# AIM-Harvard/pyradiomics

Measured on NVIDIA H100. Metric: voxels/s full-texture voxel-based, higher is better.
Workload: dtype f64

## Files before the change

### pyradiomics_b200/csrc/glcm_fast.cuh

```cuda
#pragma once
#include "vox_features.cuh"
#include "straightline.inc"
#ifndef __CUDACC__
#include <algorithm>
using std::max;
using std::min;
#endif

#ifdef __CUDA_ARCH__
#define RB_CTZ(x) (__ffs((int)(x)) - 1)
#define RB_POPC(x) __popc((unsigned)(x))
#else
#define RB_CTZ(x) __builtin_ctz((unsigned)(x))
#define RB_POPC(x) __builtin_popcount((unsigned)(x))
#endif

#if (defined(__CUDA_ARCH__) || defined(RB_EMULATE_BLOCK)) && defined(RB_GLCM_BLOCK_SYNC)
#define RB_ANGLE_SYNC() __syncthreads()
#else
#define RB_ANGLE_SYNC() ((void)0)
#endif

namespace rb {

constexpr int GF_NA = 13;
constexpr int GF_LOGT = 40;
constexpr int GF_KT = 256;
constexpr int GF_DENSE_MAX_CLS = 10;

struct GlcmFastTables {
  uint8_t orig[GF_NA];
  uint8_t np[GF_NA];
  uint8_t pA[GF_NA][18], pB[GF_NA][18];
  double log2t[GF_LOGT];
  double idm[GF_KT], idmn[GF_KT], id[GF_KT], idn[GF_KT], inv[GF_KT];
  double lz0[19];
  double rsq[GF_LOGT];
};

static const double kLanczosStart0[19] = {0.47733602246716966, 0.56675833970975287, 1.047365457332734, 0.92625467075097456, 0.641109550601909, 0.58281392786638453, 0.84830875358718982, 0.43673418560371335, 0.9227560440146213, 1.1918028652699371, 0.49824571462957101, 1.1988811518333182, 0.91723745310037241, 0.34589793559411208, 0.69183966616781278, 1.1364799193275177, 0.9474534998820221, 0.57647286407011211, 0.9839281633300665};

inline void glcm_fast_build_tables(GlcmFastTables& T, int Ng) {
  int ang[13][3], k = 0;
  for (int z = 1; z >= -1; z--) for (int y = 1; y >= -1; y--) for (int x = 1; x >= -1; x--) {
    if (k < 13) { ang[k][0] = z; ang[k][1] = y; ang[k][2] = x; k++; }
  }
  int slot = 0;
  for (int want = 1; want <= 3; want++)
    for (int a = 0; a < 13; a++) {
      int nm = (ang[a][0] != 0) + (ang[a][1] != 0) + (ang[a][2] != 0);
      if (nm != want) continue;
      T.orig[slot] = (uint8_t)a;
      int n = 0;
      for (int z = 0; z < 3; z++) for (int y = 0; y < 3; y++) for (int x = 0; x < 3; x++) {
        int z2 = z + ang[a][0], y2 = y + ang[a][1], x2 = x + ang[a][2];
        if (z2 < 0 || z2 > 2 || y2 < 0 || y2 > 2 || x2 < 0 || x2 > 2) continue;
        T.pA[slot][n] = (uint8_t)(z * 9 + y * 3 + x);
        T.pB[slot][n] = (uint8_t)(z2 * 9 + y2 * 3 + x2);
        n++;
      }
      T.np[slot] = (uint8_t)n;
      for (int t = n; t < 18; t++) { T.pA[slot][t] = 0; T.pB[slot][t] = 0; }
      slot++;
    }
  for (int i = 0; i < 19; i++) T.lz0[i] = kLanczosStart0[i];
  T.log2t[0] = 0; T.rsq[0] = 0;
  for (int c = 1; c < GF_LOGT; c++) { T.log2t[c] = log2((double)c); T.rsq[c] = 1.0 / sqrt((double)c); }
  for (int d = 0; d < GF_KT; d++) {
    double kk = d;
    T.idm[d] = 1.0 / (1.0 + kk * kk);
    T.idmn[d] = 1.0 / (1.0 + kk * kk / ((double)Ng * Ng));
    T.id[d] = 1.0 / (1.0 + kk);
    T.idn[d] = 1.0 / (1.0 + kk / (double)Ng);
    T.inv[d] = d ? 1.0 / (kk * kk) : 0.0;
  }
}

struct GlcmSolveTables {
  uint8_t np[GF_NA];
  uint8_t pA[GF_NA][18], pB[GF_NA][18];
  double lz0[19];
  double rsq[GF_LOGT];
  double rinv[GF_LOGT];
  uint32_t lo_mask[GF_NA];
  uint8_t dshift[GF_NA];
};
RB_HD void glcm_solve_tables_from(const GlcmFastTables& T, GlcmSolveTables& S) {
  for (int a = 0; a < GF_NA; a++) {
    S.np[a] = T.np[a];
    for (int t = 0; t < 18; t++) { S.pA[a][t] = T.pA[a][t]; S.pB[a][t] = T.pB[a][t]; }
    uint32_t lo = 0;
    for (int t = 0; t < T.np[a]; t++) lo |= 1u << (T.pA[a][t] < T.pB[a][t] ? T.pA[a][t] : T.pB[a][t]);
    S.lo_mask[a] = lo;
    S.dshift[a] = (uint8_t)(T.pA[a][0] < T.pB[a][0] ? T.pB[a][0] - T.pA[a][0] : T.pA[a][0] - T.pB[a][0]);
  }
  for (int i = 0; i < 19; i++) S.lz0[i] = T.lz0[i];
  for (int i = 0; i < GF_LOGT; i++) { S.rsq[i] = T.rsq[i]; S.rinv[i] = i ? 1.0 / (double)i : 0.0; }
}

#ifdef __CUDA_ARCH__
#define RB_VCMPEQ4_LSB(a, b) (__vcmpeq4((a), (b)) & 0x01010101u)
#else
static inline uint32_t rb_vcmpeq4_lsb(uint32_t a, uint32_t b) {
  const uint32_t x = a ^ b;
  const uint32_t t = ((x & 0x7F7F7F7Fu) + 0x7F7F7F7Fu) | x | 0x7F7F7F7Fu;
  return (~t) >> 7;
}
#define RB_VCMPEQ4_LSB(a, b) rb_vcmpeq4_lsb((a), (b))
#endif

RB_HD void glcm_pack_window(const uint8_t* w, int ws, uint32_t* W7) {
#pragma unroll
  for (int k = 0; k < 7; k++) {
    uint32_t v = 0;
#pragma unroll
    for (int b = 0; b < 4; b++) if (4 * k + b < 27) v |= (uint32_t)w[(4 * k + b) * ws] << (8 * b);
    W7[k] = v;
  }
}
RB_HD uint32_t glcm_eq_positions(const uint32_t* W7, uint32_t lev) {
  const uint32_t rep = lev * 0x01010101u;
  uint32_t m = 0;
#pragma unroll
  for (int k = 0; k < 7; k++) m |= ((RB_VCMPEQ4_LSB(W7[k], rep) * 0x01020408u) >> 24) << (4 * k);
  return m & 0x7FFFFFFu;
}

template <int N>
RB_HD double tridiag_bisect_static(const double* d, const double* e, double lo, double hi, int k) {
  for (int it = 0; it < 36; it++) {
    const double xm = 0.5 * (lo + hi);
    double pm2 = 1.0, pm1 = d[0] - xm;
    int cnt = pm1 <= 0;
#pragma unroll
    for (int i = 1; i < N; i++) {
      const double e2 = e[i] * e[i];
      if (e2 == 0) { pm2 = 1.0; pm1 = d[i] - xm; cnt += pm1 <= 0; continue; }
      const double p = (d[i] - xm) * pm1 - e2 * pm2;
      const bool neg_prev = pm1 < 0 || (pm1 == 0 && pm2 > 0);
      const bool neg_cur = p < 0 || (p == 0 && !neg_prev);
      cnt += neg_cur != neg_prev;
      pm2 = pm1; pm1 = p;
    }
    if (cnt > k) hi = xm; else lo = xm;
  }
  return 0.5 * (lo + hi);
}
template <int N, bool SYNC>
RB_HD void tridiag_extreme_pair_static(const double* d, const double* e, double* hi_out, double* lo_out, bool live) {
  double lo = d[0], hi = d[0];
#pragma unroll
  for (int i = 0; i < N; i++) {
    const double r = (i > 0 ? fabs(e[i]) : 0.0) + (i + 1 < N ? fabs(e[i + 1]) : 0.0);
    lo = fmin(lo, d[i] - r); hi = fmax(hi, d[i] + r);
  }
  double x[2] = {hi + 1e-9, lo - 1e-9};
  bool done[2] = {!live, !live};
  for (int it = 0; it < 24; it++) {
    const bool pending = !(done[0] && done[1]);
#if defined(__CUDA_ARCH__) || defined(RB_EMULATE_BLOCK)
    if (SYNC) { if (!__syncthreads_or(pending)) break; } else
#endif
    if (!pending) break;
#pragma unroll
    for (int c = 0; c < 2; c++) {
      double p0 = 1.0, p1 = d[0] - x[c], q0 = 0.0, q1 = -1.0, r0 = 0.0, r1 = 0.0;
#pragma unroll
      for (int i = 1; i < N; i++) {
        const double a = d[i] - x[c], b = e[i] * e[i];
        const double p2 = a * p1 - b * p0;
        const double q2 = a * q1 - p1 - b * q0;
        const double r2 = a * r1 - 2.0 * q1 - b * r0;
        p0 = p1; p1 = p2; q0 = q1; q1 = q2; r0 = r1; r1 = r2;
      }
      if (done[c]) continue;
      if (p1 == 0) { done[c] = true; continue; }
      const double G = q1 / p1, H = G * G - r1 / p1;
      const double disc = (double)(N - 1) * ((double)N * H - G * G);
      const double sq = sqrt(disc > 0 ? disc : 0.0);
      const double den = fabs(G + sq) > fabs(G - sq) ? G + sq : G - sq;
      if (den == 0 || den != den) continue;
      const double step = (double)N / den;
      x[c] -= step;
      if (fabs(step) < 1e-10) done[c] = true;
    }
  }
  *hi_out = done[0] ? x[0] : tridiag_bisect_static<N>(d, e, lo - 1e-9, hi + 1e-9, N - 1);
  *lo_out = done[1] ? x[1] : tridiag_bisect_static<N>(d, e, lo - 1e-9, hi + 1e-9, 0);
  if (!live) { *hi_out = 0; *lo_out = 0; }
}

#if defined(__CUDA_ARCH__) || defined(RB_EMULATE_BLOCK)
#define RB_SOLVE_SYNC() do { if (SYNC) __syncthreads(); } while (0)
#else
#define RB_SOLVE_SYNC() do { } while (0)
#endif
template <int N, bool SYNC = false, class TT>
RB_HD double glcm_small_solve(const uint8_t* w, int ws, const uint32_t* W7, const TT& T, int s, bool* ok, bool live = true) {
  RB_SOLVE_SYNC();
  const int dsh = T.dshift[s];
  const uint32_t NZ = ~glcm_eq_positions(W7, 0u) & 0x7FFFFFFu;
  const uint32_t VL = NZ & (NZ >> dsh) & T.lo_mask[s];
  uint32_t U = VL | (VL << dsh);
  uint32_t El[N], Eh[N];
  int R[N];
#pragma unroll
  for (int i = 0; i < N; i++) {
    uint32_t E = 0;
    if (U) { E = glcm_eq_positions(W7, w[RB_CTZ(U) * ws]); U &= ~E; }
    El[i] = E & VL;
    Eh[i] = (E >> dsh) & VL;
    R[i] = RB_POPC(El[i]) + RB_POPC(Eh[i]);
  }
  *ok = U == 0;
  if (!SYNC && U) return 0.0;
  if (U) live = false;
  RB_SOLVE_SYNC();
  const double invS = 1.0 / (2.0 * RB_POPC(VL));
  double v1[N], rs[N];
#pragma unroll
  for (int i = 0; i < N; i++) { rs[i] = T.rsq[R[i]]; v1[i] = sqrt(R[i] * invS); }
  double a[N][N];
#pragma unroll
  for (int i = 0; i < N; i++)
#pragma unroll
    for (int j = 0; j <= i; j++) {
      const int c = (i == j) ? 2 * RB_POPC(El[i] & Eh[i]) : RB_POPC(El[i] & Eh[j]) + RB_POPC(El[j] & Eh[i]);
      a[i][j] = c * rs[i] * rs[j] - v1[i] * v1[j];
    }
  double d[N], e[N];
  e[0] = 0;
#pragma unroll
  for (int k = 0; k + 2 < N; k++) {
    RB_SOLVE_SYNC();
    double sigma = 0;
#pragma unroll
    for (int i = k + 2; i < N; i++) sigma += a[i][k] * a[i][k];
    const double x0 = a[k + 1][k];
    d[k] = a[k][k];
    if (sigma < 1e-30) { e[k + 1] = x0; continue; }
    const double nrm = sqrt(x0 * x0 + sigma);
    const double alpha = x0 > 0 ? -nrm : nrm;
    double v[N], pv[N];
    v[k + 1] = x0 - alpha;
#pragma unroll
    for (int i = k + 2; i < N; i++) v[i] = a[i][k];
    const double beta = -1.0 / (alpha * v[k + 1]);
    double K = 0;
#pragma unroll
    for (int i = k + 1; i < N; i++) {
      double acc = 0;
#pragma unroll
      for (int j = k + 1; j < N; j++) acc += (j <= i ? a[i][j] : a[j][i]) * v[j];
      pv[i] = beta * acc;
      K += v[i] * pv[i];
    }
    K *= 0.5 * beta;
#pragma unroll
    for (int i = k + 1; i < N; i++) pv[i] -= K * v[i];
#pragma unroll
    for (int i = k + 1; i < N; i++)
#pragma unroll
      for (int j = k + 1; j <= i; j++) a[i][j] -= v[i] * pv[j] + pv[i] * v[j];
    e[k + 1] = alpha;
  }
  d[N - 2] = a[N - 2][N - 2]; e[N - 1] = a[N - 1][N - 2]; d[N - 1] = a[N - 1][N - 1];
  double hi, lo;
  RB_SOLVE_SYNC();
  tridiag_extreme_pair_static<N, SYNC>(d, e, &hi, &lo, live);
  return fmax(fabs(hi), fabs(lo));
}

}
#include "glcm_lanczos.cuh"
namespace rb {

template <class TT>
RB_HD double glcm_lanczos_solve(const uint8_t* w, int ws, const TT& T, int s, int cls, double* sm, int st) {
  if (s > 2) return 1.0;
  int n = 0;
  double r;
  if (cls <= 12) r = glcm_lanczos_task<14>(w, ws, T, s, sm, st, &n);
  else if (cls <= 14) r = glcm_lanczos_task<16>(w, ws, T, s, sm, st, &n);
  else { r = glcm_lanczos_task<18>(w, ws, T, s, sm, st, &n); if (n == 19) r = 1.0; }
  return r;
}

template <class TT>
RB_HD double glcm_fast_solve(const uint8_t* w, int ws, const TT& T, int s, int cls) {
  if (cls <= GF_DENSE_MAX_CLS) {
    uint32_t W7[7];
    glcm_pack_window(w, ws, W7);
    bool ok = false;
    double r;
    if (cls <= 2) r = glcm_small_solve<4>(w, ws, W7, T, s, &ok);
    else if (cls <= 4) r = glcm_small_solve<6>(w, ws, W7, T, s, &ok);
    else if (cls <= 6) r = glcm_small_solve<8>(w, ws, W7, T, s, &ok);
    else if (cls <= 8) r = glcm_small_solve<10>(w, ws, W7, T, s, &ok);
    else r = glcm_small_solve<12>(w, ws, W7, T, s, &ok);
    return ok ? r : NAN;
  }
  double sm[LZ_NARR * 18];
  return glcm_lanczos_solve(w, ws, T, s, cls, sm, 1);
}

constexpr int GF_NCLS = 16, GF_CLS_BITS = 4;
RB_HD int glcm_task_class(int n) { return n <= 2 ? 0 : n >= 17 ? 15 : n - 2; }

struct GlcmAcc {
  double sum[GLCM_NF];
  int n_ok, n_imc2;
  uint32_t tasks;
  unsigned long long tcls;
  bool ja_nan;
};

#ifdef __CUDA_ARCH__
#define RB_VMINU2(a, b) __vminu2((a), (b))
#define RB_VMAXU2(a, b) __vmaxu2((a), (b))
#else
static inline uint32_t rb_vminu2(uint32_t a, uint32_t b) {
  return min(a >> 16, b >> 16) << 16 | min(a & 0xFFFFu, b & 0xFFFFu);
}
static inline uint32_t rb_vmaxu2(uint32_t a, uint32_t b) {
  return max(a >> 16, b >> 16) << 16 | max(a & 0xFFFFu, b & 0xFFFFu);
}
#define RB_VMINU2(a, b) rb_vminu2((a), (b))
#define RB_VMAXU2(a, b) rb_vmaxu2((a), (b))
#endif

template <int NP, bool FULL>
RB_HD void glcm_fast_angle(const uint8_t* w, int ws, const uint32_t* eq, int es,
                           const GlcmFastTables& T, int s, const VoxParams& P, GlcmAcc& acc) {
  const uint8_t* pA = T.pA[s];
  const uint8_t* pB = T.pB[s];
  const int dsh = (int)pB[0] - (int)pA[0];
  uint32_t key[NP];
  uint32_t valid = 0, EA = 0, EB = 0;
  int n = 0, Ssum = 0, Sab = 0, Sq = 0, Skd = 0;
  bool selfpair = false;
#pragma unroll
  for (int t = 0; t < NP; t++) {
    const int a = w[pA[t] * ws], b = w[pB[t] * ws];
    const bool ok = FULL || (a != 0 && b != 0);
    const int kd = a > b ? a - b : b - a, ks = a + b;
    key[t] = ok ? (uint32_t)(ks << 16 | kd) : 0xFFFFFFFFu;
    if (ok) {
      valid |= 1u << t; EA |= 1u << pA[t]; EB |= 1u << pB[t];
      n++; Ssum += ks; Sab += a * b; Sq += a * a + b * b; Skd += kd;
      selfpair |= kd == 0;
    }
  }
  const int orig = T.orig[s];
  if (!FULL && n == 0) {
    if (P.alive[orig >> 5] >> (orig & 31) & 1u) acc.ja_nan = true;
    return;
  }
  double rl = 0, lgE = 0;
  int E2 = 0, cmax = 0;
  uint32_t reps = 0, all = 0, comp = 0;
  uint32_t em[NP];
#pragma unroll
  for (int t = 0; t < NP; t++) {
    em[t] = 0;
    if (valid >> t & 1u) {
      const uint32_t ea = eq[pA[t] * es], eb = eq[pB[t] * es];
      rl += T.log2t[RB_POPC(ea & EA) + RB_POPC(ea & EB)] + T.log2t[RB_POPC(eb & EA) + RB_POPC(eb & EB)];
      reps |= (ea & (0u - ea)) | (eb & (0u - eb));
      em[t] = ea | eb;
      all |= em[t];
      if (!comp) comp = em[t];
      const int c = RB_POPC(((ea & (eb >> dsh)) | (eb & (ea >> dsh))) & EA);
      const int cc = ea == eb ? 2 * c : c;
      lgE += T.log2t[cc];
      E2 += 2 * cc;
      cmax = cc > cmax ? cc : cmax;
    }
  }
  const int nlev = RB_POPC(reps);
  double mcc;
  if (P.n_roi_levels < 2) mcc = 1.0;
  else if (nlev < 2) mcc = 0.0;
  else {
    for (int sweep = 0; sweep < NP; sweep++) {
      const uint32_t before = comp;
#pragma unroll
      for (int t = 0; t < NP; t++) if (em[t] & comp) comp |= em[t];
      if (comp == before) break;
    }
    bool bipartite = false;
    if (comp == all && !selfpair) {
      bool connected;
      glcm_graph_scan(eq, es, EA, dsh, EA | EB, false, &connected, &bipartite, true);
    }
    if (comp != all || bipartite) mcc = 1.0;
    else {
      mcc = 0.0; acc.tasks |= 1u << s;
      acc.tcls |= (unsigned long long)glcm_task_class(nlev) << (GF_CLS_BITS * s);
    }
  }
  if (NP == 18) RB_SORTNET2x16_18(key);
  else if (NP == 12) RB_SORTNET2x16_12(key);
  else RB_SORTNET2x16_8(key);
  const int S2 = 2 * n;
  const double S = (double)S2, invS = 1.0 / S, invS2 = invS * invS;
  const double ux = Ssum * invS;
  const double ac = 2.0 * Sab * invS;
  const double contrast = 2.0 * (double)(Sq - 2 * Sab) * invS;
  const int vnum = S2 * Sq - Ssum * Ssum;
  const double sxx = vnum * invS2;
  const double sxy = (double)(2 * Sab * S2 - Ssum * Ssum) * invS2;
  const double ct = (double)(2 * (Sq + 2 * Sab) * S2 - 4 * Ssum * Ssum) * invS2;
  const double da = 2.0 * Skd * invS;
  const double dvar = (double)(2 * (Sq - 2 * Sab) * S2 - 4 * Skd * Skd) * invS2;
  double cs = 0, cp = 0, idm = 0, idmn = 0, id = 0, idn = 0, inv = 0, lgD = 0, lgS = 0;
  int startS = 0, startD = 0;
#pragma unroll
  for (int i = 0; i < NP; i++) {
    if (FULL || i < n) {
      const int ks = (int)(key[i] >> 16), kd = (int)(key[i] & 0xFFFFu);
      const double dn = (double)(ks * n - Ssum), d2 = dn * dn;
      cs += d2 * dn; cp += d2 * d2;
      const uint32_t nx = (i + 1 < NP) ? key[i + 1 < NP ? i + 1 : i] : 0xFFFFFFFFu;
      const bool last = (i + 1 == n);
      const int runS = (last || (int)(nx >> 16) != ks) ? i + 1 - startS : 0;
      const int runD = (last || (int)(nx & 0xFFFFu) != kd) ? i + 1 - startD : 0;
      lgS += runS * T.log2t[2 * runS];
      const double r = (double)runD;
      lgD += r * T.log2t[2 * runD];
      idm += r * T.idm[kd]; idmn += r * T.idmn[kd]; id += r * T.id[kd]; idn += r * T.idn[kd]; inv += r * T.inv[kd];
      startS = runS ? i + 1 : startS;
      startD = runD ? i + 1 : startD;
    }
  }
  const double invn = 1.0 / n, invn2 = invn * invn;
  const double lS = T.log2t[2 * n];
  const double hxy = -2.0 * invS * (lgE - n * lS);
  const double dent = -2.0 * invS * (lgD - n * lS);
  const double sent = -2.0 * invS * (lgS - n * lS);
  const double hx0 = nlev > 1 ? lS - rl * invS : 0.0;
  const double hx = hx0, hxy2 = 2.0 * hx0, hxy1 = hxy2;
  double f[GLCM_NF];
  f[G_Autocorrelation] = ac; f[G_JointAverage] = ux;
  f[G_ClusterProminence] = cp * invn2 * invn2 * invn; f[G_ClusterShade] = cs * invn2 * invn2; f[G_ClusterTendency] = ct;
  f[G_Contrast] = contrast;
  f[G_Correlation] = (vnum == 0) ? 1.0 : sxy / (sxx + EPS);
  f[G_DifferenceAverage] = da; f[G_DifferenceEntropy] = dent; f[G_DifferenceVariance] = dvar;
  f[G_JointEnergy] = E2 * invS2; f[G_JointEntropy] = hxy;
  f[G_Imc1] = (hx != 0) ? (hxy - hxy1) / hx : 0.0;
  const double dxy = hxy2 - hxy;
  f[G_Imc2] = (fabs(dxy) < 1e-12) ? 0.0 : sqrt(1.0 - exp(-2.0 * dxy));
  f[G_Idm] = 2.0 * idm * invS; f[G_Idmn] = 2.0 * idmn * invS; f[G_Id] = 2.0 * id * invS; f[G_Idn] = 2.0 * idn * invS;
  f[G_InverseVariance] = 2.0 * inv * invS;
  f[G_MaximumProbability] = cmax * invS; f[G_SumAverage] = 2.0 * ux; f[G_SumEntropy] = sent; f[G_SumSquares] = sxx;
  f[G_MCC] = mcc;
#pragma unroll
  for (int k = 0; k < GLCM_NF; k++) if (k != G_Imc2) acc.sum[k] += f[k];
  acc.n_ok++;
  if (f[G_Imc2] == f[G_Imc2]) { acc.sum[G_Imc2] += f[G_Imc2]; acc.n_imc2++; }
}

template <bool FULL = false>
RB_HD uint32_t glcm_fast_voxel_phaseA(const uint8_t* w, int ws, uint32_t* eq, int es, const GlcmFastTables& T,
                                      const VoxParams& P, double* out, int* n_ok_out, unsigned long long* tcls_out = nullptr) {
  uint32_t e[27];
  int wl[27];
#pragma unroll
  for (int p = 0; p < 27; p++) wl[p] = w[p * ws];
  if (FULL) RB_EQMASKS_27_KEY(wl, e);
  else RB_EQMASKS_27(wl, e);
#pragma unroll
  for (int p = 0; p < 27; p++) eq[p * es] = e[p];
  GlcmAcc acc;
#pragma unroll
  for (int k = 0; k < GLCM_NF; k++) acc.sum[k] = 0;
  acc.n_ok = 0; acc.n_imc2 = 0; acc.ja_nan = false; acc.tasks = 0; acc.tcls = 0;
  for (int s = 0; s < 3; s++) { if (!FULL) RB_ANGLE_SYNC(); glcm_fast_angle<18, FULL>(w, ws, eq, es, T, s, P, acc); }
  for (int s = 3; s < 9; s++) { if (!FULL) RB_ANGLE_SYNC(); glcm_fast_angle<12, FULL>(w, ws, eq, es, T, s, P, acc); }
  for (int s = 9; s < 13; s++) { if (!FULL) RB_ANGLE_SYNC(); glcm_fast_angle<8, FULL>(w, ws, eq, es, T, s, P, acc); }
  *n_ok_out = acc.n_ok;
  if (tcls_out) *tcls_out = acc.tcls;
  const double inv = acc.n_ok ? 1.0 / acc.n_ok : NAN;
#pragma unroll
  for (int k = 0; k < GLCM_NF; k++) out[k] = acc.n_ok ? acc.sum[k] * inv : NAN;
  out[G_Imc2] = acc.n_imc2 ? acc.sum[G_Imc2] / acc.n_imc2 : NAN;
  if (acc.ja_nan) out[G_JointAverage] = NAN;
  return acc.tasks;
}

RB_HD double glcm_fast_finish_mcc(double partial_mean, int n_ok, uint32_t tasks, const double* solved, int ss) {
  double add = 0;
  for (int s = 0; s < GF_NA; s++) if (tasks >> s & 1u) add += solved[s * ss];
  return n_ok ? partial_mean + add / n_ok : partial_mean;
}

RB_HD bool glcm_window_full(const uint8_t* w, int ws) {
  bool full = true;
#pragma unroll
  for (int p = 0; p < 27; p++) full &= w[p * ws] != 0;
  return full;
}

RB_HD void glcm_fast_voxel(const uint8_t* w, int ws, uint32_t* eq, int es, const GlcmFastTables& T,
                           const VoxParams& P, double* out) {
  int n_ok = 0;
  unsigned long long tcls = 0;
  const uint32_t tasks = glcm_window_full(w, ws) ? glcm_fast_voxel_phaseA<true>(w, ws, eq, es, T, P, out, &n_ok, &tcls)
                                                 : glcm_fast_voxel_phaseA<false>(w, ws, eq, es, T, P, out, &n_ok, &tcls);
  double solved[GF_NA];
  GlcmSolveTables ST;
  glcm_solve_tables_from(T, ST);
  for (int s = 0; s < GF_NA; s++) solved[s] = (tasks >> s & 1u) ? glcm_fast_solve(w, ws, ST, s, (int)(tcls >> (GF_CLS_BITS * s) & (GF_NCLS - 1))) : 0.0;
  out[G_MCC] = glcm_fast_finish_mcc(out[G_MCC], n_ok, tasks, solved, 1);
}

}
```

### pyradiomics_b200/csrc/glcm_lanczos.cuh

```cuda
#pragma once

namespace rb {

constexpr uint32_t LZ_LOW = 0x36DB6DBu;
constexpr int LZ_ACC = 3;
constexpr int LZ_NARR = 5;
constexpr double GF_BREAKDOWN = 1e-10;

RB_HD constexpr int lz_smem_doubles(int N) { return LZ_NARR * N; }

template <int N, class TT>
RB_HD double glcm_lanczos_axis(const int* wl, const TT& T, double* sm, int st, int* n_out, bool live = true) {
  double* const U = sm;
  double* const S = sm + (size_t)N * st;
  double* const IR = sm + (size_t)2 * N * st;
  double* const D = sm + (size_t)3 * N * st;
  double* const E = sm + (size_t)4 * N * st;
  uint32_t W7[7];
#pragma unroll
  for (int k = 0; k < 7; k++) {
    uint32_t v = 0;
#pragma unroll
    for (int b = 0; b < 4; b++) if (4 * k + b < 27) v |= (uint32_t)wl[4 * k + b] << (8 * b);
    W7[k] = v;
  }
  const uint32_t NZ = ~glcm_eq_positions(W7, 0u) & 0x7FFFFFFu;
  const uint32_t VL = NZ & (NZ >> 1) & LZ_LOW;
  const uint32_t VH = VL << 1;
  uint32_t Urem = VL | VH;
  double Rd[N];
  uint32_t plane[5] = {0, 0, 0, 0, 0};
  int n = 0;
#pragma unroll
  for (int i = 0; i < N; i++) {
    uint32_t Ec = 0;
    if (Urem) {
      const int p = RB_CTZ(Urem);
      const uint32_t lev = (W7[p >> 2] >> (8 * (p & 3))) & 255u;
      Ec = glcm_eq_positions(W7, lev);
      Urem &= ~Ec;
      n++;
    }
    const int Ri = RB_POPC(Ec & VL) + RB_POPC(Ec & VH);
    Rd[i] = (double)Ri;
    IR[(size_t)i * st] = T.rinv[Ri];
#pragma unroll
    for (int b = 0; b < 5; b++) if (i >> b & 1) plane[b] |= Ec;
  }
  *n_out = n + (Urem ? RB_POPC(Urem) : 0);
  if (Urem) return NAN;
  uint32_t ida[3] = {0, 0, 0}, idb[3] = {0, 0, 0};
#pragma unroll
  for (int t = 0; t < 18; t++) {
    const int p = (t / 2) * 3 + (t % 2);
    uint32_t a = 0, b = 0;
#pragma unroll
    for (int k = 0; k < 5; k++) { a |= ((plane[k] >> p) & 1u) << k; b |= ((plane[k] >> (p + 1)) & 1u) << k; }
    ida[t / 6] |= a << (5 * (t % 6));
    idb[t / 6] |= b << (5 * (t % 6));
  }
  double y0[N], y1[N];
  double Ssum = 0, dot = 0;
#pragma unroll
  for (int i = 0; i < N; i++) {
    y1[i] = Rd[i] != 0.0 ? T.lz0[i] : 0.0;
    y0[i] = 0.0;
    Ssum += Rd[i];
    dot += Rd[i] * y1[i];
  }
  const double cc = 1.0 / Ssum;
  double nrm = 0;
  {
    const double sh = dot * cc;
#pragma unroll
    for (int i = 0; i < N; i++) { y1[i] = Rd[i] != 0.0 ? y1[i] - sh : 0.0; nrm += Rd[i] * y1[i] * y1[i]; }
  }
  {
    const double inrm = 1.0 / sqrt(nrm);
#pragma unroll
    for (int i = 0; i < N; i++) y1[i] *= inrm;
  }
  double beta = 0;
  E[0] = 0;
  for (int j = 0; j < N - 1; j++) {
#pragma unroll
    for (int i = 0; i < N; i++) { U[(size_t)i * st] = y1[i]; S[(size_t)i * st] = 0.0; }
#pragma unroll
    for (int t = 0; t < 18; t++) {
      const int p = (t / 2) * 3 + (t % 2);
      if (VL >> p & 1u) {
        const size_t a = (size_t)((ida[t / 6] >> (5 * (t % 6))) & 31u) * st, b = (size_t)((idb[t / 6] >> (5 * (t % 6))) & 31u) * st;
        const double ua = U[a], ub = U[b];
        S[a] += ub;
        S[b] += ua;
      }
    }
    double al[LZ_ACC];
#pragma unroll
    for (int k = 0; k < LZ_ACC; k++) al[k] = 0;
#pragma unroll
    for (int i = 0; i < N; i++) {
      const double s = S[(size_t)i * st];
      al[i % LZ_ACC] += y1[i] * s;
      y0[i] = s * IR[(size_t)i * st] - beta * y0[i];
    }
    double alpha = 0;
#pragma unroll
    for (int k = 0; k < LZ_ACC; k++) alpha += al[k];
    double dvp[LZ_ACC], c1p[LZ_ACC];
#pragma unroll
    for (int k = 0; k < LZ_ACC; k++) { dvp[k] = 0; c1p[k] = 0; }
#pragma unroll
    for (int i = 0; i < N; i++) {
      y0[i] -= alpha * y1[i];
      const double g = Rd[i] * y0[i];
      dvp[i % LZ_ACC] += g; c1p[i % LZ_ACC] += g * y1[i];
    }
    double dv = 0, c1 = 0;
#pragma unroll
    for (int k = 0; k < LZ_ACC; k++) { dv += dvp[k]; c1 += c1p[k]; }
    dv *= cc;
    double nbp[LZ_ACC];
#pragma unroll
    for (int k = 0; k < LZ_ACC; k++) nbp[k] = 0;
#pragma unroll
    for (int i = 0; i < N; i++) {
      const double zi = Rd[i] != 0.0 ? y0[i] - dv - c1 * y1[i] : 0.0;
      y0[i] = zi;
      nbp[i % LZ_ACC] += Rd[i] * zi * zi;
    }
    double nb = 0;
#pragma unroll
    for (int k = 0; k < LZ_ACC; k++) nb += nbp[k];
    D[(size_t)j * st] = alpha;
    nb = sqrt(nb);
    const bool ok = nb > GF_BREAKDOWN;
    const double inb = ok ? 1.0 / nb : 0.0;
    beta = ok ? nb : 0.0;
    if (j + 1 < N - 1) E[(size_t)(j + 1) * st] = beta;
#pragma unroll
    for (int i = 0; i < N; i++) { const double t1 = y1[i]; y1[i] = y0[i] * inb; y0[i] = t1; }
  }
  double d[N - 1], e[N - 1];
#pragma unroll
  for (int i = 0; i < N - 1; i++) { d[i] = D[(size_t)i * st]; e[i] = E[(size_t)i * st]; }
  double hi, lo;
  tridiag_extreme_pair_static<N - 1, false>(d, e, &hi, &lo, live && n >= 2);
  return fmax(fabs(hi), fabs(lo));
}

template <int N, class TT>
RB_HD double glcm_lanczos_task(const uint8_t* w, int ws, const TT& T, int s, double* sm, int st, int* n_out, bool live = true) {
  int wl[27];
#pragma unroll
  for (int a = 0; a < 3; a++)
#pragma unroll
    for (int b = 0; b < 3; b++)
#pragma unroll
      for (int c = 0; c < 3; c++) {
        const int v2 = w[(a * 9 + b * 3 + c) * ws], v1 = w[(a * 9 + c * 3 + b) * ws], v0 = w[(c * 9 + a * 3 + b) * ws];
        wl[a * 9 + b * 3 + c] = s == 2 ? v2 : s == 1 ? v1 : v0;
      }
  return glcm_lanczos_axis<N>(wl, T, sm, st, n_out, live);
}

RB_HD void glcm_graph_scan(const uint32_t* eq, int es, uint32_t EA, int dsh, uint32_t U, bool selfpair, bool* connected,
                           bool* bipartite, bool stop_at_odd_cycle = false) {
  const int p0 = RB_CTZ(EA);
  if (selfpair) {
    uint32_t Cm = eq[(size_t)p0 * es], F = Cm;
    while (F) {
      uint32_t Pn = (((F & EA) << dsh) | ((F >> dsh) & EA)) & ~Cm;
      F = 0;
      while (Pn) { const uint32_t c = eq[(size_t)RB_CTZ(Pn) * es]; F |= c; Pn &= ~c; }
      Cm |= F;
    }
    *connected = (U & ~Cm) == 0;
    *bipartite = false;
    return;
  }
  uint32_t CA = eq[(size_t)p0 * es], CB = 0, FA = CA, FB = 0;
  while (FA | FB) {
    uint32_t PA = (((FA & EA) << dsh) | ((FA >> dsh) & EA)) & ~CB;
    uint32_t PB = (((FB & EA) << dsh) | ((FB >> dsh) & EA)) & ~CA;
    FA = 0; FB = 0;
    while (PA) { const uint32_t c = eq[(size_t)RB_CTZ(PA) * es]; FB |= c; PA &= ~c; }
    while (PB) { const uint32_t c = eq[(size_t)RB_CTZ(PB) * es]; FA |= c; PB &= ~c; }
    CA |= FA; CB |= FB;
    if (stop_at_odd_cycle && (CA & CB)) break;
  }
  *connected = (U & ~(CA | CB)) == 0;
  *bipartite = (CA & CB) == 0;
}

}
```

Measured before the change: 264.6 million.

## Restructure Lanczos sparse matvec per line and clamp eigen search bounds

Replaces the 18-edge scatter (read both endpoints, add to S) with a per-line 3-node gather that writes each node's sum once, using a first-position mask to zero S on first touch instead of a separate clearing pass. This drops the per-iteration zeroing stores and the read-modify-write chains on shared memory. The Newton/bisection start for the tridiagonal extreme eigenvalues is also clamped to [-1,1], since the normalized matrix's spectrum lies there, so fewer iterations should be needed. The matvec now depends on a correct node index per position and on masking S for unused rows.

```diff
diff --git a/pyradiomics_b200/csrc/glcm_fast.cuh b/pyradiomics_b200/csrc/glcm_fast.cuh
--- a/pyradiomics_b200/csrc/glcm_fast.cuh
+++ b/pyradiomics_b200/csrc/glcm_fast.cuh
@@ -147,14 +147,15 @@
   return 0.5 * (lo + hi);
 }
 template <int N, bool SYNC>
-RB_HD void tridiag_extreme_pair_static(const double* d, const double* e, double* hi_out, double* lo_out, bool live) {
+RB_HD void tridiag_extreme_pair_static(const double* d, const double* e, double* hi_out, double* lo_out, bool live,
+                                       double bound = INFINITY) {
   double lo = d[0], hi = d[0];
 #pragma unroll
   for (int i = 0; i < N; i++) {
     const double r = (i > 0 ? fabs(e[i]) : 0.0) + (i + 1 < N ? fabs(e[i + 1]) : 0.0);
     lo = fmin(lo, d[i] - r); hi = fmax(hi, d[i] + r);
   }
-  double x[2] = {hi + 1e-9, lo - 1e-9};
+  double x[2] = {fmin(hi, bound) + 1e-9, fmax(lo, -bound) - 1e-9};
   bool done[2] = {!live, !live};
   for (int it = 0; it < 24; it++) {
     const bool pending = !(done[0] && done[1]);
diff --git a/pyradiomics_b200/csrc/glcm_lanczos.cuh b/pyradiomics_b200/csrc/glcm_lanczos.cuh
--- a/pyradiomics_b200/csrc/glcm_lanczos.cuh
+++ b/pyradiomics_b200/csrc/glcm_lanczos.cuh
@@ -8,6 +8,7 @@
 constexpr double GF_BREAKDOWN = 1e-10;
 
 RB_HD constexpr int lz_smem_doubles(int N) { return LZ_NARR * N; }
+RB_HD size_t lz_node(const uint32_t* NW, int p) { return (NW[p / 6] >> (5 * (p % 6))) & 31u; }
 
 template <int N, class TT>
 RB_HD double glcm_lanczos_axis(const int* wl, const TT& T, double* sm, int st, int* n_out, bool live = true) {
@@ -30,6 +31,7 @@
   uint32_t Urem = VL | VH;
   double Rd[N];
   uint32_t plane[5] = {0, 0, 0, 0, 0};
+  uint32_t FP = 0;
   int n = 0;
 #pragma unroll
   for (int i = 0; i < N; i++) {
@@ -39,6 +41,7 @@
       const uint32_t lev = (W7[p >> 2] >> (8 * (p & 3))) & 255u;
       Ec = glcm_eq_positions(W7, lev);
       Urem &= ~Ec;
+      FP |= Ec & (0u - Ec);
       n++;
     }
     const int Ri = RB_POPC(Ec & VL) + RB_POPC(Ec & VH);
@@ -49,15 +52,13 @@
   }
   *n_out = n + (Urem ? RB_POPC(Urem) : 0);
   if (Urem) return NAN;
-  uint32_t ida[3] = {0, 0, 0}, idb[3] = {0, 0, 0};
-#pragma unroll
-  for (int t = 0; t < 18; t++) {
-    const int p = (t / 2) * 3 + (t % 2);
-    uint32_t a = 0, b = 0;
-#pragma unroll
-    for (int k = 0; k < 5; k++) { a |= ((plane[k] >> p) & 1u) << k; b |= ((plane[k] >> (p + 1)) & 1u) << k; }
-    ida[t / 6] |= a << (5 * (t % 6));
-    idb[t / 6] |= b << (5 * (t % 6));
+  uint32_t NW[5] = {0, 0, 0, 0, 0};
+#pragma unroll
+  for (int p = 0; p < 27; p++) {
+    uint32_t a = 0;
+#pragma unroll
+    for (int k = 0; k < 5; k++) a |= ((plane[k] >> p) & 1u) << k;
+    NW[p / 6] |= a << (5 * (p % 6));
   }
   double y0[N], y1[N];
   double Ssum = 0, dot = 0;
@@ -84,15 +85,18 @@
   E[0] = 0;
   for (int j = 0; j < N - 1; j++) {
 #pragma unroll
-    for (int i = 0; i < N; i++) { U[(size_t)i * st] = y1[i]; S[(size_t)i * st] = 0.0; }
-#pragma unroll
-    for (int t = 0; t < 18; t++) {
-      const int p = (t / 2) * 3 + (t % 2);
-      if (VL >> p & 1u) {
-        const size_t a = (size_t)((ida[t / 6] >> (5 * (t % 6))) & 31u) * st, b = (size_t)((idb[t / 6] >> (5 * (t % 6))) & 31u) * st;
-        const double ua = U[a], ub = U[b];
-        S[a] += ub;
-        S[b] += ua;
+    for (int i = 0; i < N; i++) U[(size_t)i * st] = y1[i];
+#pragma unroll
+    for (int l = 0; l < 9; l++) {
+      const int p = 3 * l;
+      const bool va = VL >> p & 1u, vb = VL >> (p + 1) & 1u;
+      const double ya = U[lz_node(NW, p) * st], yb = U[lz_node(NW, p + 1) * st], yc = U[lz_node(NW, p + 2) * st];
+      const double z[3] = {va ? yb : 0.0, (va ? ya : 0.0) + (vb ? yc : 0.0), vb ? yb : 0.0};
+#pragma unroll
+      for (int c = 0; c < 3; c++) {
+        double* const s = &S[lz_node(NW, p + c) * st];
+        const double old = *s;
+        *s = (FP >> (p + c) & 1u ? 0.0 : old) + z[c];
       }
     }
     double al[LZ_ACC];
@@ -100,7 +104,7 @@
     for (int k = 0; k < LZ_ACC; k++) al[k] = 0;
 #pragma unroll
     for (int i = 0; i < N; i++) {
-      const double s = S[(size_t)i * st];
+      const double s = Rd[i] != 0.0 ? S[(size_t)i * st] : 0.0;
       al[i % LZ_ACC] += y1[i] * s;
       y0[i] = s * IR[(size_t)i * st] - beta * y0[i];
     }
@@ -145,7 +149,7 @@
 #pragma unroll
   for (int i = 0; i < N - 1; i++) { d[i] = D[(size_t)i * st]; e[i] = E[(size_t)i * st]; }
   double hi, lo;
-  tridiag_extreme_pair_static<N - 1, false>(d, e, &hi, &lo, live && n >= 2);
+  tridiag_extreme_pair_static<N - 1, false>(d, e, &hi, &lo, live && n >= 2, 1.0);
   return fmax(fabs(hi), fabs(lo));
 }
 
```

New measurement: 269.7 million (median of 6 runs). 1.9% higher.
